# volume-em/empanada-napari

Measured on AMD Instinct MI355X. Metric: EM tiles/sec (1024^2 fp16), higher is better.
Workload: dtype f16

## Files before the change

empanada-napari_amd/csrc/common.h:

```cpp
#pragma once
#include <hip/hip_runtime.h>
#include <stdint.h>
#include <stdio.h>
#include <string>

#include "../../include/empanada_hip.h"

typedef _Float16 half_t;
typedef _Float16 f16x8 __attribute__((ext_vector_type(8)));
typedef _Float16 f16x4 __attribute__((ext_vector_type(4)));
typedef _Float16 f16x2 __attribute__((ext_vector_type(2)));
typedef float f32x4 __attribute__((ext_vector_type(4)));

namespace emp {

void set_error(const char* fmt, ...);

#define EMP_CHECK_HIP(expr)                                                        \
  do {                                                                             \
    hipError_t _e = (expr);                                                        \
    if (_e != hipSuccess) {                                                        \
      emp::set_error("%s:%d: %s -> %s", __FILE__, __LINE__, #expr, hipGetErrorString(_e)); \
      return EMP_ERR_HIP;                                                          \
    }                                                                              \
// ... 22 lines not shown
  const float* bias;
  const float* bias_n;
  const half_t* res;
  half_t* out;
  const half_t* zero;
  int N, H, W, Cin, in_ld;
  int Cout, KH, KW, stride, pad, dil;
  int Ho, Wo, out_ld, res_ld;
  int act;
  int ps_cout;
  int M;
  int mt, nt;
  int mt_per_xcd;
  int kgroup;
  int ngroup;
  const half_t* in2;
  int Cin2, in2_ld, H2, W2, stride2;
  half_t* out2;
  int out2_ld, split;
  half_t* out3;
  int out3_ld, split3;
  const half_t* next_w;
  const float* next_b;
  half_t* next_out;
  int next_cout, next_ld;
};

int launch_conv_igemm(const ConvParams& p, int variant, hipStream_t stream);
int launch_conv_igemm_grouped(const ConvParams& p, int groups, int gs_in, long long gs_w, int gs_out, hipStream_t stream);
bool conv_igemm256_supported(const ConvParams& p);
bool conv_uses_256(const ConvParams& p);
int launch_conv_igemm256(ConvParams p, hipStream_t stream, int kg = 0, int mode = 0, bool wpacked = false);
int conv256_pack_kgroup(int KT, int Cin);
int conv256_pack_weights(const half_t* w, half_t* out, int Cout, int KT, int Cin, int Cin2, hipStream_t stream);
bool conv_b2b_supported(const ConvParams& p);
bool conv_igemm_h256_supported(const ConvParams& p);
int launch_conv_igemm_h256(ConvParams p, hipStream_t stream, int kg = 0);
bool conv_igemm_s64_supported(const ConvParams& p);
int launch_conv_igemm_s64(ConvParams p, hipStream_t stream, int kg = 0);
bool conv3x3_c64_supported(const ConvParams& p);
int launch_conv3x3_c64(const ConvParams& p, hipStream_t stream);

int launch_stem7x7(const void* img, int dtype, float sub, float mul, int N, int H, int W, int vh, int vw,
                   const float* w , const float* b , half_t* out, hipStream_t s);
int launch_maxpool3x3s2(const half_t* in, int N, int H, int W, int C, half_t* out, hipStream_t s);
int launch_stem3x3s2_f16(const void* img, int dtype, float sub, float mul, int N, int H, int W, int vh, int vw,
                         const float* w , const float* b, int C, half_t* out, int out_ld, hipStream_t s);
int launch_gate_mul_f16(const half_t* x, int x_ld, half_t* g , int g_ld, int64_t rows, int C,
                        hipStream_t s);
int launch_stem_pool(const void* img, int dtype, float sub, float mul, int N, int H, int W, int vh, int vw,
                     const float* w, const float* b, half_t* out, hipStream_t s);
int launch_stem_pool_f32(const void* img, int dtype, float sub, float mul, int N, int H, int W, int vh, int vw,
                         const float* w, const float* b, float* out, hipStream_t s);
int launch_dwconv(const half_t* in, int N, int H, int W, int C, int in_ld, const half_t* w, int K,
                  half_t* out, int out_ld, const half_t* zero, hipStream_t s);
int launch_fuse_combine(const half_t* a, const half_t* b, const half_t* c, float ca, float cb, float cc, int mode,
                        int N, int H, int W, int C, half_t* out, hipStream_t s, half_t* out_lo = nullptr, int out_ld = 0);
int launch_bilinear_ac(const half_t* in, int N, int h, int w, int C, int in_ld, half_t* out, int H, int W,
                       int out_ld, hipStream_t s);
int launch_avgpool(const half_t* in, int N, int HW, int C, int in_ld, float* out , float* part,
                   hipStream_t s);
int avgpool_scratch_floats(int N, int C);
int launch_gemv(const float* in, int N, int K, const float* w, const float* b, int Cout, int relu,
                float* out, hipStream_t s);
bool sepconv5_supported(int C, int Cout, int head_c);
int launch_sepconv5_pack_pw(const half_t* w, int pw_ld, int C, int Cout, half_t* packed, hipStream_t s);
// ... 97 lines not shown
```

empanada-napari_amd/csrc/conv_igemm.hip:

```cpp
#include "common.h"

#ifdef EMP_IGEMM_GROUPED
#define EMP_IGEMM_KARGS const ConvParams p_, const int gs_in, const long long gs_w, const int gs_out
#define EMP_IGEMM_KPROLOGUE                                                \
  ConvParams p = p_;                                                       \
  {                                                                        \
    const int g_ = blockIdx.y;                                             \
    p.in += (size_t)g_ * gs_in;                                            \
    p.wgt += (size_t)g_ * (size_t)gs_w;                                    \
    p.out += (size_t)g_ * gs_out;                                          \
    if (p.bias) p.bias += (size_t)g_ * gs_out;                             \
  }
#else
#define EMP_IGEMM_KARGS const ConvParams p
#define EMP_IGEMM_KPROLOGUE
#endif

#include <type_traits>

namespace emp {

namespace {

constexpr int BK = 64;
// ... 387 lines not shown
  ConvParams q = p;
  {
    const int CB = p.Cin / 64, KT = p.KH * p.KW;
    int kg = (KT > 1 && CB > 4 && CB % 4 == 0) ? 4 : CB;
    q.kgroup = kg;
  }
  if (p.Cout <= 64 || cdiv(p.Cout, 64) * 64 <= cdiv(p.Cout, 128) * 128)
    return launch_grouped_tpl<128, 64, 2, 2, true, true, 3>(q, groups, gs_in, gs_w, gs_out, stream);
  return launch_grouped_tpl<128, 128, 2, 2, true, true>(q, groups, gs_in, gs_w, gs_out, stream);
}

#else
template <int BM, int BN, int WPM, int WPN, bool GLDS, bool EPI_LDS, int OCC = 2>
int launch_tpl(ConvParams p, hipStream_t stream) {
  p.mt = cdiv(p.M, BM);
  p.nt = cdiv(p.Cout, BN);
  p.mt_per_xcd = cdiv(p.mt, 8);
  const int grid = 8 * p.mt_per_xcd * p.nt;
  hipLaunchKernelGGL((conv_igemm_kernel<BM, BN, WPM, WPN, GLDS, EPI_LDS, OCC>), dim3(grid), dim3(256), 0, stream, p);
  EMP_LAUNCH_CHECK();
  return EMP_OK;
}

}

bool conv_uses_256(const ConvParams& p) {
  static const bool no256 = [] { const char* e = getenv("EMP_CONV_NO256"); return e && e[0] == '1'; }();
  static const int min_k = [] { const char* e = getenv("EMP_CONV_256_MINK"); return e ? atoi(e) : 512; }();
  const int64_t tiles256 = (int64_t)cdiv(p.M, 256) * (p.Cout / 256);
  const int k256 = p.KH * p.KW * p.Cin + (p.in2 ? p.Cin2 : 0);
  const bool out2_ok = !p.out2 || (!p.out3 && p.split % 256 == 0);
  return !no256 && out2_ok && conv_igemm256_supported(p) && tiles256 >= 192 && k256 >= (p.in2 ? min_k / 4 : min_k);
}
bool conv_uses_h256(const ConvParams& p) {
  static const int h256 = [] { const char* e = getenv("EMP_CONV_H256"); return e ? atoi(e) : 1; }();
  if (!h256 || !conv_igemm_h256_supported(p)) return false;
  const int64_t tiles = (int64_t)cdiv(p.M, 128) * (p.Cout / 128) / 2;
  if (tiles < 1024) return false;
  return h256 == 2 || (p.Cout == 128 && p.KH * p.KW * p.Cin >= 256);
}

int launch_conv_igemm(const ConvParams& p, int variant, hipStream_t stream) {
  EMP_REQUIRE(p.Cin % BK == 0 && p.Cin > 0, "conv: Cin=%d must be a positive multiple of 64", p.Cin);
  EMP_REQUIRE(p.in_ld % 8 == 0 && p.in_ld >= p.Cin, "conv: in_ld=%d must be >= Cin and a multiple of 8", p.in_ld);
  EMP_REQUIRE(p.Cout % 8 == 0 && p.Cout > 0, "conv: Cout=%d must be a positive multiple of 8", p.Cout);
  EMP_REQUIRE(p.out_ld % 8 == 0 && p.out_ld >= (p.ps_cout ? p.ps_cout : (p.out2 ? p.split : p.Cout)), "conv: out_ld=%d invalid", p.out_ld);
  EMP_REQUIRE(p.ps_cout == 0 || (p.ps_cout % 8 == 0 && p.Cout == 4 * p.ps_cout && p.res == nullptr),
              "conv: pixel-shuffle store needs Cout == 4*ps_cout, ps_cout %% 8 == 0, no residual");
  EMP_REQUIRE(p.act >= 0 && p.act <= 2, "conv: act must be 0 (none), 1 (ReLU) or 2 (SiLU)");
  EMP_REQUIRE(p.res == nullptr || p.res_ld % 8 == 0, "conv: res_ld=%d must be a multiple of 8", p.res_ld);
  EMP_REQUIRE(((uintptr_t)p.in % 16) == 0 && ((uintptr_t)p.out % 16) == 0 && ((uintptr_t)p.wgt % 16) == 0 &&
                  ((uintptr_t)p.res % 16) == 0 && ((uintptr_t)p.zero % 256) == 0 && p.zero != nullptr,
              "conv: pointers must be 16-byte aligned (zero page 256)");
  EMP_REQUIRE((int64_t)p.N * p.Ho * p.Wo < (1ll << 31), "conv: too many output pixels");
  if (p.out2) {
    EMP_REQUIRE(p.split > 0 && p.split < p.Cout && p.split % 8 == 0 && p.out2_ld % 8 == 0 &&
                    p.out2_ld >= (p.out3 ? p.split3 : p.Cout) - p.split &&
                    p.out_ld >= p.split && ((uintptr_t)p.out2 % 16) == 0 && p.ps_cout == 0 && p.res == nullptr,
                "conv: second destination: split=%d must be a multiple of 8 inside (0, Cout=%d)", p.split, p.Cout);
  }
  if (p.out3) {
    EMP_REQUIRE(p.out2 != nullptr && p.split3 > p.split && p.split3 < p.Cout && p.split3 % 8 == 0 && p.out3_ld % 8 == 0 &&
                    p.out3_ld >= p.Cout - p.split3 && ((uintptr_t)p.out3 % 16) == 0,
                "conv: third destination: split3=%d must be a multiple of 8 inside (split=%d, Cout=%d)", p.split3, p.split, p.Cout);
  }
  if (p.in2) {
    EMP_REQUIRE(p.KH == 1 && p.KW == 1 && p.stride == 1 && p.pad == 0,
                "conv: a second source needs a 1x1 / stride 1 main convolution");
    EMP_REQUIRE(p.Cin2 > 0 && p.Cin2 % BK == 0 && p.in2_ld % 8 == 0 && p.in2_ld >= p.Cin2 && ((uintptr_t)p.in2 % 16) == 0,
                "conv: second source: Cin2=%d must be a positive multiple of 64, in2_ld=%d >= Cin2", p.Cin2, p.in2_ld);
    EMP_REQUIRE(p.stride2 >= 1 && (p.Ho - 1) * p.stride2 < p.H2 && (p.Wo - 1) * p.stride2 < p.W2,
                "conv: second source %dx%d / stride %d does not cover the %dx%d output", p.H2, p.W2, p.stride2, p.Ho, p.Wo);
  }
  int v = variant & 15, tile = (variant >> 4) & 15, kg = (variant >> 8) & 255, mode256 = (variant >> 16) & 15;
  if ((variant >> 20) & 1) {
    EMP_REQUIRE(!p.next_w && conv_igemm256_supported(p), "conv: packed weights belong to the 256x256 tile");
    return launch_conv_igemm256(p, stream, 0, mode256, true);
  }
  if (p.next_w) {
    EMP_REQUIRE(conv_b2b_supported(p), "conv: a fused next convolution needs the 256x256 tile (Cout == 256, >= 192 tiles)");
    return launch_conv_igemm256(p, stream, kg, mode256);
  }
  EMP_REQUIRE(v <= 3 && tile <= 7, "conv: bad variant %d", variant);
  if (tile == 7) return launch_conv_igemm_s64(p, stream, kg);
  if (tile == 6) return launch_conv3x3_c64(p, stream);
  if (tile == 5) return launch_conv_igemm_h256(p, stream, kg);
  {
    static const bool no_c64 = [] { const char* e = getenv("EMP_CONV_NO_C64"); return e && e[0] == '1'; }();
    if (tile == 0 && !no_c64 && conv3x3_c64_supported(p) && (int64_t)p.N * cdiv(p.H, 8) * cdiv(p.W, 16) >= 1024)
      return launch_conv3x3_c64(p, stream);
  }
  if (tile == 4) {
    return launch_conv_igemm256(p, stream, kg, mode256);
  }
  ConvParams q = p;
  {
    const int CB = p.Cin / 64, KT = p.KH * p.KW;
    static const int env_kg = [] { const char* e = getenv("EMP_CONV_KGROUP"); return e ? atoi(e) : 0; }();
    if (kg == 0) kg = env_kg;
    if (kg == 0) kg = (KT > 1 && CB > 4 && CB % 4 == 0) ? 4 : CB;
    if (kg > CB || CB % kg != 0 || KT == 1) kg = CB;
    q.kgroup = kg;
  }
  if (tile == 0) {
    if (conv_uses_256(p)) return launch_conv_igemm256(p, stream);
    if (conv_uses_h256(p)) return launch_conv_igemm_h256(p, stream);
    tile = (p.Cout <= 64) ? 2 : 1;
    if (p.Cout > 128 && cdiv(p.Cout, 64) * 64 < cdiv(p.Cout, 128) * 128) tile = 2;
    static const int small_below = [] { const char* e = getenv("EMP_CONV_SMALL_TILES_BELOW"); return e ? atoi(e) : 256; }();
// ... 26 lines not shown
```

empanada-napari_amd/csrc/conv_igemm256.hip:

```cpp
#include "common.h"

namespace emp {

namespace {

constexpr int KS = 32;
constexpr int SLOT_BYTES = 512 * 64;
constexpr int W_OFF = 256 * 64;
constexpr int NSLOT = 4;

__device__ __forceinline__ int perm32b(int x) {
  const int t = x >> 4, i = x & 15;
  return ((i >> 2) << 3) + (t << 2) + (i & 3);
}
__device__ __forceinline__ void lds_barrier() {
  asm volatile("s_waitcnt lgkmcnt(0)\n\ts_barrier" ::: "memory");
}

template <int ACT>
__device__ __forceinline__ float act_c(float x) {
  if (ACT == 1) return fmaxf(x, 0.f);
  if (ACT == 2) return x / (1.f + __expf(-x));
  return x;
}
// ... 22 lines not shown
      rv[q][0] = *reinterpret_cast<const f16x8*>(rp);
      rv[q][1] = *reinterpret_cast<const f16x8*>(m < p.M ? rp + 32 : p.zero);
    }
  }
#pragma unroll
  for (int q = 0; q < 8; ++q) {
    const int m = mrow0 + q * 16 + fr;
    if (m >= p.M) continue;
    half_t* orow = (p.out2 && co0 >= p.split) ? p.out2 + (size_t)m * p.out2_ld + (co0 - p.split) + fq * 8
                                              : p.out + (size_t)m * p.out_ld + co0 + fq * 8;
    const float* bn = p.bias_n ? p.bias_n + (size_t)(m / HoWo) * p.Cout + co0 + fq * 8 : nullptr;
#pragma unroll
    for (int P = 0; P < 2; ++P) {
      float v[8];
#pragma unroll
      for (int r = 0; r < 4; ++r) {
        v[r] = acc[2 * P][q][r] + bv[P][r];
        v[4 + r] = acc[2 * P + 1][q][r] + bv[P][4 + r];
      }
      if (bn) {
        const float4 b0 = *reinterpret_cast<const float4*>(bn + P * 32);
        const float4 b1 = *reinterpret_cast<const float4*>(bn + P * 32 + 4);
        v[0] += b0.x; v[1] += b0.y; v[2] += b0.z; v[3] += b0.w;
        v[4] += b1.x; v[5] += b1.y; v[6] += b1.z; v[7] += b1.w;
      }
      if (p.res) {
#pragma unroll
        for (int r = 0; r < 8; ++r) v[r] += (float)rv[q][P][r];
      }
      f16x8 o;
#pragma unroll
      for (int r = 0; r < 8; ++r) o[r] = (half_t)act_c<ACT>(v[r]);
      *reinterpret_cast<f16x8*>(orow + P * 32) = o;
    }
  }
}
template <int ACT>
__device__ __forceinline__ void wave_epilogue_b2b(const ConvParams& p, f32x4 (&acc)[4][8], char* lds, int m0, int grp, int wc,
                                                  int wave, int fr, int fq, int HoWo) {
  const int mrow0 = m0 + grp * 128, co0 = wc * 64;
  float bv[2][8];
#pragma unroll
  for (int P = 0; P < 2; ++P) {
    const int co = co0 + P * 32 + fq * 8;
#pragma unroll
    for (int r = 0; r < 8; ++r) bv[P][r] = 0.f;
    if (p.bias) {
      const float4 b0 = *reinterpret_cast<const float4*>(p.bias + co);
      const float4 b1 = *reinterpret_cast<const float4*>(p.bias + co + 4);
      bv[P][0] = b0.x; bv[P][1] = b0.y; bv[P][2] = b0.z; bv[P][3] = b0.w;
      bv[P][4] = b1.x; bv[P][5] = b1.y; bv[P][6] = b1.z; bv[P][7] = b1.w;
    }
  }
  f16x8 rv[8][2];
  if (p.res) {
#pragma unroll
    for (int q = 0; q < 8; ++q) {
      const int m = mrow0 + q * 16 + fr;
      const half_t* rp = m < p.M ? p.res + (size_t)m * p.res_ld + co0 + fq * 8 : p.zero;
      rv[q][0] = *reinterpret_cast<const f16x8*>(rp);
      rv[q][1] = *reinterpret_cast<const f16x8*>(m < p.M ? rp + 32 : p.zero);
    }
  }
#pragma unroll
  for (int q = 0; q < 8; ++q) {
    const int row = grp * 128 + q * 16 + fr;
// ... 27 lines not shown
#pragma unroll
    for (int tp = 0; tp < 2; ++tp)
#pragma unroll
      for (int t = 0; t < 2; ++t) a2[tp][t] = f32x4{0.f, 0.f, 0.f, 0.f};
    const int r0 = pp * 32 + perm32b(fr), r1 = pp * 32 + perm32b(16 + fr);
#pragma unroll
    for (int ks = 0; ks < 8; ++ks) {
      const f16x8 wa = *reinterpret_cast<const f16x8*>(w2 + r0 * 512 + (((ks * 4 + fq) ^ (r0 & 15)) << 4));
      const f16x8 wb = *reinterpret_cast<const f16x8*>(w2 + r1 * 512 + (((ks * 4 + fq) ^ (r1 & 15)) << 4));
#pragma unroll
      for (int t = 0; t < 2; ++t) {
        const int row = wave * 32 + t * 16 + fr;
        const f16x8 yb = *reinterpret_cast<const f16x8*>(lds + row * 512 + (((ks * 4 + fq) ^ (row & 15)) << 4));
        a2[0][t] = __builtin_amdgcn_mfma_f32_16x16x32_f16(wa, yb, a2[0][t], 0, 0, 0);
        a2[1][t] = __builtin_amdgcn_mfma_f32_16x16x32_f16(wb, yb, a2[1][t], 0, 0, 0);
      }
    }
    const int co2 = pp * 32 + fq * 8;
    const float4 b0 = *reinterpret_cast<const float4*>(p.next_b + co2);
    const float4 b1 = *reinterpret_cast<const float4*>(p.next_b + co2 + 4);
#pragma unroll
    for (int t = 0; t < 2; ++t) {
      const int m = m0 + wave * 32 + t * 16 + fr;
      if (m >= p.M) continue;
      f16x8 o;
      o[0] = (half_t)fmaxf(a2[0][t][0] + b0.x, 0.f); o[1] = (half_t)fmaxf(a2[0][t][1] + b0.y, 0.f);
      o[2] = (half_t)fmaxf(a2[0][t][2] + b0.z, 0.f); o[3] = (half_t)fmaxf(a2[0][t][3] + b0.w, 0.f);
      o[4] = (half_t)fmaxf(a2[1][t][0] + b1.x, 0.f); o[5] = (half_t)fmaxf(a2[1][t][1] + b1.y, 0.f);
      o[6] = (half_t)fmaxf(a2[1][t][2] + b1.z, 0.f); o[7] = (half_t)fmaxf(a2[1][t][3] + b1.w, 0.f);
      *reinterpret_cast<f16x8*>(p.next_out + (size_t)m * p.next_ld + co2) = o;
    }
  }
}
__device__ __forceinline__ void wave_epilogue_any(const ConvParams& p, f32x4 (&acc)[4][8], int mrow0, int co0, int fr,
                                                  int fq, int HoWo) {
  if (p.act == 1) wave_epilogue<1>(p, acc, mrow0, co0, fr, fq, HoWo);
  else if (p.act == 2) wave_epilogue<2>(p, acc, mrow0, co0, fr, fq, HoWo);
  else wave_epilogue<0>(p, acc, mrow0, co0, fr, fq, HoWo);
}

#ifdef EMP_CLOCK_STAMP
__device__ unsigned long long emp_clock_stamp_buf[2 * 8192];
#endif

template <int DMA_EARLY, bool B2B>
__global__ void __launch_bounds__(512, 1) conv_igemm256_kernel(const ConvParams p) {
  extern __shared__ __attribute__((aligned(1024))) char lds[];
#ifdef EMP_CLOCK_STAMP
  const unsigned long long stamp_c0 = __builtin_amdgcn_s_memtime(), stamp_r0 = __builtin_amdgcn_s_memrealtime();
#endif

  const int bid = blockIdx.x;
  const int xcd = bid & 7, j = bid >> 3;
  int mtile = xcd * p.mt_per_xcd + j / p.nt;
  int ntile = j % p.nt;
  if (p.ngroup > 0) {
    const int per = p.mt_per_xcd * p.ngroup, g = j / per, rem = j - g * per;
    mtile = xcd * p.mt_per_xcd + rem / p.ngroup;
    ntile = g * p.ngroup + rem % p.ngroup;
  }
  if (mtile >= p.mt) return;
  const int m0 = mtile * 256, n0 = ntile * 256;

  const int tid = threadIdx.x, l = tid & 63;
  const int wave = __builtin_amdgcn_readfirstlane(tid >> 6);
  const int grp = wave >> 2, wc = wave & 3;
  const int HoWo = p.Ho * p.Wo;
  const int KT = p.KH * p.KW;
// ... 619 lines not shown

  stage();
  if (KTOT > 1) {
    stage();
    asm volatile("s_waitcnt vmcnt(6)" ::: "memory");
  } else {
    asm volatile("s_waitcnt vmcnt(0)" ::: "memory");
  }
  lds_barrier();

  f16x8 pf[8], wf[4];
  for (int t = 0; t < KTOT; ++t) {
    const char* base = lds + (t % 3) * HSLOT;
#pragma unroll
    for (int c = 0; c < 4; ++c) wf[c] = *reinterpret_cast<const f16x8*>(base + w_off + c * 1024);
#pragma unroll
    for (int q = 0; q < 8; ++q) pf[q] = *reinterpret_cast<const f16x8*>(base + p_off + q * 1024);
    if (t + 2 < KTOT) {
      stage();
      asm volatile("s_waitcnt vmcnt(6) lgkmcnt(0)" ::: "memory");
    } else {
      asm volatile("s_waitcnt vmcnt(0) lgkmcnt(0)" ::: "memory");
    }
    __builtin_amdgcn_sched_barrier(0);
    asm volatile("s_barrier" ::: "memory");
    __builtin_amdgcn_s_setprio(1);
#pragma unroll
    for (int q = 0; q < 8; ++q)
#pragma unroll
      for (int c = 0; c < 4; ++c) acc[c][q] = __builtin_amdgcn_mfma_f32_16x16x32_f16(wf[c], pf[q], acc[c][q], 0, 0, 0);
    __builtin_amdgcn_s_setprio(0);
    __builtin_amdgcn_sched_barrier(0);
  }
  wave_epilogue_any(p, acc, m0 + wp * 128, n0 + wc * 64, fr, fq, HoWo);
}

}

bool conv_b2b_supported(const ConvParams& p) {
  return p.next_w != nullptr && p.Cout == 256 && p.next_cout == 64 &&
         p.next_ld % 8 == 0 && p.ps_cout == 0 && p.out2 == nullptr && p.bias_n == nullptr && p.act <= 1 &&
         (int64_t)cdiv(p.M, 256) >= 192 && p.Cin % KS == 0 && (!p.in2 || p.Cin2 % KS == 0);
}

bool conv_igemm256_supported(const ConvParams& p) {
  return p.Cout % 256 == 0 && p.ps_cout == 0 && p.Cin % KS == 0 && p.KH * p.KW * (p.Cin / KS) + (p.in2 ? p.Cin2 / KS : 0) >= 1;
}

__global__ void __launch_bounds__(256) pack256_kernel(const half_t* __restrict__ w, half_t* __restrict__ out, int Cout, int KT,
                                                      int Cin, int Cin2, int KG) {
  const int CB = Cin / KS, KT1 = KT * CB, KTOT = KT1 + Cin2 / KS, Krow = KT * Cin + Cin2;
  const int64_t total = (int64_t)(Cout / 256) * KTOT * 16 * 64;
  for (int64_t i = (int64_t)blockIdx.x * 256 + threadIdx.x; i < total; i += (int64_t)gridDim.x * 256) {
    const int l = (int)(i & 63), pc = (int)((i >> 6) & 15);
    const int64_t tt = i >> 10;
    const int t = (int)(tt % KTOT), ntile = (int)(tt / KTOT);
    const int row = pc * 16 + (l >> 2);
    const int co = ntile * 256 + (row & ~31) + perm32b(row & 31);
    const int chunk = (l & 3) ^ ((-(l >> 4)) & 3);
    int koff;
    if (t < KT1) {
      const int per = KT * KG, g = t / per, idx = t - g * per, tap = idx / KG, cb = idx - tap * KG;
      koff = tap * Cin + (g * KG + cb) * KS;
    } else {
      koff = KT * Cin + (t - KT1) * KS;
    }
    *reinterpret_cast<uint4*>(out + i * 8) = *reinterpret_cast<const uint4*>(w + (size_t)co * Krow + koff + chunk * 8);
  }
}

template <int DMA_EARLY, bool B2B = false>
static int launch256(const ConvParams& p, int grid, hipStream_t stream) {
  constexpr int LDS_BYTES = NSLOT * SLOT_BYTES + (B2B ? 64 * 256 * 2 : 0);
  if (int rc = ensure_dyn_lds(reinterpret_cast<const void*>(&conv_igemm256_kernel<DMA_EARLY, B2B>), LDS_BYTES)) return rc;
  hipLaunchKernelGGL((conv_igemm256_kernel<DMA_EARLY, B2B>), dim3(grid), dim3(512), LDS_BYTES, stream, p);
  EMP_LAUNCH_CHECK();
  return EMP_OK;
}

int launch_conv_igemm256(ConvParams p, hipStream_t stream, int kg, int mode, bool wpacked) {
  EMP_REQUIRE(conv_igemm256_supported(p), "conv256: unsupported shape (Cout=%d)", p.Cout);
  EMP_REQUIRE(p.next_w == nullptr || conv_b2b_supported(p), "conv256: the fused next convolution needs Cout == 256 (got %d)", p.Cout);
  EMP_REQUIRE(p.out2 == nullptr || (p.split % 256 == 0 && p.split > 0 && p.split < p.Cout && p.out3 == nullptr &&
                                    p.next_w == nullptr && p.out2_ld % 8 == 0 && p.out2_ld >= p.Cout - p.split),
              "conv256: a second destination takes whole 256-cout tiles (split=%d)", p.split);
  {
    const int CB = p.Cin / KS, KT = p.KH * p.KW;
    static const int env_kg = [] { const char* e = getenv("EMP_CONV256_KGROUP"); return e ? atoi(e) : 0; }();
    if (kg == 0) kg = env_kg;
    if (kg == 0) kg = 8;
    if (KT == 1 || kg > CB || CB % kg != 0) kg = CB;
    p.kgroup = kg;
  }
  if (wpacked) {
    EMP_REQUIRE(p.next_w == nullptr && p.kgroup == conv256_pack_kgroup(p.KH * p.KW, p.Cin), "conv256: packed weights need the default K walk");
    p.kgroup = -p.kgroup;
  }
  static const int env_mode = [] { const char* e = getenv("EMP_CONV256_MODE"); return e ? atoi(e) : 0; }();
  if (mode == 0) mode = env_mode;
  p.mt = cdiv(p.M, 256);
  p.nt = p.Cout / 256;
  p.mt_per_xcd = cdiv(p.mt, 8);
  {
    static const int env_ng = [] { const char* e = getenv("EMP_CONV256_NGROUP"); return e ? atoi(e) : 0; }();
    p.ngroup = (env_ng > 0 && p.KH * p.KW == 1 && p.nt >= 2 * env_ng && p.nt % env_ng == 0 && !p.next_w) ? env_ng : 0;
  }
  const int grid = 8 * p.mt_per_xcd * p.nt;
  if (p.next_w) return launch256<0, true>(p, grid, stream);
  {
    static const bool wide_on = [] { const char* e = getenv("EMP_CONV256_WIDE"); return !(e && e[0] == '0'); }();
    const int kga = p.kgroup < 0 ? -p.kgroup : p.kgroup;
    const int ktot = p.KH * p.KW * (p.Cin / KS) + (p.in2 ? p.Cin2 / KS : 0);
    if (wide_on && mode == 0 && p.Cin % (2 * KS) == 0 && (!p.in2 || p.Cin2 % (2 * KS) == 0) && kga % 2 == 0 && ktot >= 8 &&
        (int64_t)p.N * p.H * p.W < (1ll << 31)) {
      if (int rc = ensure_dyn_lds(reinterpret_cast<const void*>(&conv_igemm256w_kernel), WIDE_LDS_BYTES)) return rc;
      hipLaunchKernelGGL(conv_igemm256w_kernel, dim3(grid), dim3(512), WIDE_LDS_BYTES, stream, p);
      EMP_LAUNCH_CHECK();
      return EMP_OK;
    }
  }
  if (mode == 1) return launch256<2>(p, grid, stream);
  if (mode == 2) return launch256<4>(p, grid, stream);
  return launch256<0>(p, grid, stream);
}

int conv256_pack_kgroup(int KT, int Cin) {
  const int CB = Cin / KS;
  static const int env_kg = [] { const char* e = getenv("EMP_CONV256_KGROUP"); return e ? atoi(e) : 0; }();
  int kg = env_kg ? env_kg : 8;
  if (KT == 1 || kg > CB || CB % kg != 0) kg = CB;
  return kg;
}
int conv256_pack_weights(const half_t* w, half_t* out, int Cout, int KT, int Cin, int Cin2, hipStream_t stream) {
  EMP_REQUIRE(w && out && Cout > 0 && Cout % 256 == 0 && Cin > 0 && Cin % KS == 0 && Cin2 >= 0 && Cin2 % KS == 0 && KT >= 1,
              "conv256_pack_weights: bad shape (Cout=%d Cin=%d Cin2=%d)", Cout, Cin, Cin2);
  const int64_t chunks = (int64_t)Cout * (KT * Cin + Cin2) / 8;
  hipLaunchKernelGGL(pack256_kernel, dim3((unsigned)std::min<int64_t>((chunks + 255) / 256, 4096)), dim3(256), 0, stream, w, out, Cout,
                     KT, Cin, Cin2, conv256_pack_kgroup(KT, Cin));
  EMP_LAUNCH_CHECK();
  return EMP_OK;
}

bool conv_igemm_h256_supported(const ConvParams& p) {
  return p.Cout % 128 == 0 && p.ps_cout == 0 && p.out2 == nullptr && p.Cin % KS == 0 && (!p.in2 || p.Cin2 % KS == 0);
}

template <int PXR, int COR>
static int launch_h256(ConvParams p, hipStream_t stream) {
  constexpr int LDS_BYTES = 3 * (PXR + COR) * 64;
  if (int rc = ensure_dyn_lds(reinterpret_cast<const void*>(&conv_igemm_h256_kernel<PXR, COR>), LDS_BYTES)) return rc;
  p.mt = cdiv(p.M, PXR);
  p.nt = p.Cout / COR;
  p.mt_per_xcd = cdiv(p.mt, 8);
  const int grid = 8 * p.mt_per_xcd * p.nt;
  hipLaunchKernelGGL((conv_igemm_h256_kernel<PXR, COR>), dim3(grid), dim3(256), LDS_BYTES, stream, p);
  EMP_LAUNCH_CHECK();
  return EMP_OK;
}

int launch_conv_igemm_h256(ConvParams p, hipStream_t stream, int kg) {
  EMP_REQUIRE(conv_igemm_h256_supported(p), "conv h256: unsupported shape (Cout=%d)", p.Cout);
  const int CB = p.Cin / KS, KT = p.KH * p.KW;
  if (kg == 0) kg = 8;
  if (KT == 1 || kg > CB || CB % kg != 0) kg = CB;
  p.kgroup = kg;
  if (p.Cout % 256 == 0) return launch_h256<128, 256>(p, stream);
  return launch_h256<256, 128>(p, stream);
}

// ... 9 lines not shown
```

empanada-napari_amd/csrc/pdl_net.hip:

```cpp
#include <string.h>

#include <array>
#include <map>
#include <memory>
#include <string>
#include <vector>

#include "common.h"

namespace emp {

namespace {

struct HostParam {
  std::vector<int64_t> shape;
  std::vector<float> w, b;
  bool set = false;
};

struct Act {
  half_t* p = nullptr;
  int N = 0, H = 0, W = 0, C = 0, ld = 0;
  size_t off = 0;
};

struct DevConv {
  half_t* w = nullptr;
  half_t* w256 = nullptr;
  float* b = nullptr;
  int cout = 0, cin = 0, cin_pad = 0, kh = 1, kw = 1;
  int cin2 = 0, cin2_pad = 0;
  bool wsplit = false;
};

inline int round_up(int a, int b) { return (a + b - 1) / b * b; }

}
}

using namespace emp;

struct emp_pdl {
  emp_pdl_config cfg;
  int aspp_ch = 256, dec_ch = 256, ncls = 1;
  std::vector<std::string> param_names;
  std::map<std::string, HostParam> params;
  bool finalized = false;
  FILE* layer_log = [] { const char* e = getenv("EMP_LAYER_LOG"); return e ? fopen(e, "w") : (FILE*)nullptr; }();
  bool fuse_stem = [] { const char* e = getenv("EMP_FUSE_STEM"); return !(e && e[0] == '0'); }();
  bool fuse_ds = [] { const char* e = getenv("EMP_FUSE_DS"); return !(e && e[0] == '0'); }();
  bool fuse_b2b = [] { const char* e = getenv("EMP_FUSE_B2B"); return !(e && e[0] == '0'); }();
  bool pack256 = [] { const char* e = getenv("EMP_CONV256_PACK"); return !(e && e[0] == '0'); }();
  bool fuse_proj = [] { const char* e = getenv("EMP_FUSE_PROJ"); return !(e && e[0] == '0'); }();
  bool fuse_aspp = [] { const char* e = getenv("EMP_FUSE_ASPP"); return !(e && e[0] == '0'); }();
  bool fuse_sepconv = [] { const char* e = getenv("EMP_FUSE_SEPCONV"); return !(e && e[0] == '0'); }();
  bool fuse_pr = [] { const char* e = getenv("EMP_FUSE_PR"); return !(e && e[0] == '0'); }();
  int precise_sepconv = [] { const char* e = getenv("EMP_PRECISE_SEPCONV"); return e ? atoi(e) : 1; }();
  bool precise_wsplit = [] { const char* e = getenv("EMP_PRECISE_WSPLIT"); return !(e && e[0] == '0'); }();
  bool precise_fsplit = [] { const char* e = getenv("EMP_PRECISE_FSPLIT"); return !(e && e[0] == '0'); }();
  int sepconv_min_tiles = [] { const char* e = getenv("EMP_SEPCONV_MIN_TILES"); return e ? atoi(e) : 256; }();

  int precision = [] {
    const char* e = getenv("EMP_PRECISION");
    if (e && (!strcmp(e, "fp16") || !strcmp(e, "16"))) return 0;
    if (e && (!strcmp(e, "fp32") || !strcmp(e, "32"))) return 1;
    return 2;
  }();
  bool fp32_graph() const { return precision != 0; }
  bool x3_fuse_ds = [] { const char* e = getenv("EMP_X3_FUSE_DS"); return !(e && e[0] == '0'); }();
  bool x3_fuse_head = [] { const char* e = getenv("EMP_X3_FUSE_HEAD"); return !(e && e[0] == '0'); }();
  bool x3_planes = [] { const char* e = getenv("EMP_X3_PLANES"); return !(e && e[0] == '0'); }();
  int x3_planes_min_tiles = [] { const char* e = getenv("EMP_X3_PLANES_MIN_TILES"); return e ? atoi(e) : 128; }();
  bool x3_planes_ready = false;
  bool x3_ksplit = [] { const char* e = getenv("EMP_X3_KSPLIT"); return !(e && e[0] == '0'); }();
  float* x3_kpart = nullptr;
  bool x3_small_aspp = [] { const char* e = getenv("EMP_X3_SMALL_ASPP"); return !(e && e[0] == '0'); }();
  bool x3_fuse_stem = [] { const char* e = getenv("EMP_X3_FUSE_STEM"); return !(e && e[0] == '0'); }();
  bool x3_merge_proj = [] { const char* e = getenv("EMP_X3_MERGE_PROJ"); return !(e && e[0] == '0'); }();
  bool x3_merge_aspp = [] { const char* e = getenv("EMP_X3_MERGE_ASPP"); return !(e && e[0] == '0'); }();
  bool x3_fuse_sep = [] { const char* e = getenv("EMP_X3_FUSE_SEP"); return !(e && e[0] == '0'); }();
  int x3_sep_min_tiles = [] { const char* e = getenv("EMP_X3_SEP_MIN_TILES"); return e ? atoi(e) : 1; }();
  struct SepX3 { float* dw = nullptr; half_t* pw = nullptr; int C = 0, Cout = 0, ks = 0; };
  std::map<std::string, SepX3> sepx3;
  bool regnet_grouped = [] { const char* e = getenv("EMP_REGNET_GROUPED"); return !(e && e[0] == '0'); }();
  int64_t regnet_group_tiles = [] { const char* e = getenv("EMP_REGNET_GROUP_TILES"); return e ? atoll(e) : 2048ll; }();
// ... 593 lines not shown
  p.N = in.N; p.H = in.H; p.W = in.W; p.Cin = dc.cin_pad; p.in_ld = in.ld;
  p.Cout = dc.cout; p.KH = dc.kh; p.KW = dc.kw; p.stride = stride; p.pad = pad; p.dil = dil;
  p.Ho = (in.H + 2 * pad - dil * (dc.kh - 1) - 1) / stride + 1;
  p.Wo = (in.W + 2 * pad - dil * (dc.kw - 1) - 1) / stride + 1;
  const int up = ps_cout ? 2 : 1;
  EMP_REQUIRE(p.Ho * up == out.H && p.Wo * up == out.W && in.N == out.N, "%s: output shape mismatch (%dx%d vs %dx%d)",
              wname.c_str(), p.Ho * up, p.Wo * up, out.H, out.W);
  EMP_REQUIRE(in_coff + dc.cin_pad <= in.ld && out_coff + (ps_cout ? ps_cout : (out2 ? split : dc.cout)) <= out.ld,
              "%s: channel slice out of range", wname.c_str());
  p.out_ld = out.ld;
  p.act = act;
  p.ps_cout = ps_cout;
  p.M = p.N * p.Ho * p.Wo;
  double next_flops = 0.0;
  if (fused_next) *fused_next = false;
  if (next_name && n->fuse_b2b) {
    const DevConv& nd = n->convs.at(*next_name);
    p.next_w = nd.w; p.next_b = nd.b; p.next_out = next_out->p; p.next_cout = nd.cout; p.next_ld = next_out->ld;
    if (nd.kh == 1 && nd.kw == 1 && nd.cin_pad == dc.cout && nd.cin2_pad == 0 && next_out->N == out.N && next_out->H == out.H &&
        next_out->W == out.W && nd.cout <= next_out->ld && out_coff == 0 && conv_b2b_supported(p)) {
      *fused_next = true;
      next_flops = 2.0 * (double)p.M * nd.cout * (double)nd.cin;
      n->flops += next_flops;
    } else {
      p.next_w = nullptr; p.next_b = nullptr; p.next_out = nullptr; p.next_cout = 0; p.next_ld = 0;
    }
  }
  const double kflop = (double)(dc.cin * dc.kh * dc.kw + (dc.wsplit ? 0 : dc.cin2));
  n->flops += 2.0 * (double)p.M * dc.cout * kflop;
  if (n->layer_log)
    fprintf(n->layer_log, "conv,%s,%d,%d,%d,%d,%d,%d,%d,%d\n", wname.c_str(), p.M, dc.cin_pad + dc.cin2_pad, dc.cout, dc.kh,
            stride, dil, res ? 1 : 0, in.N * in.H * in.W);
  int variant = 0;
  if (n->pack256 && !p.next_w && conv_uses_256(p)) {
    if (dc.w256) {
      p.wgt = dc.w256;
      variant = 1 << 20;
    }
  }
  if (n->profile && !p.next_w && conv_uses_256(p)) {
    if (n->prof_used == n->prof_events.size()) {
      hipEvent_t a, b;
      EMP_CHECK_HIP(hipEventCreate(&a));
      EMP_CHECK_HIP(hipEventCreate(&b));
      n->prof_events.emplace_back(a, b);
    }
    auto& ev = n->prof_events[n->prof_used++];
    EMP_CHECK_HIP(hipEventRecord(ev.first, s));
    const int rc = launch_conv_igemm(p, variant, s);
    EMP_CHECK_HIP(hipEventRecord(ev.second, s));
    n->prof_flops += 2.0 * (double)p.M * dc.cout * kflop;
    return rc;
  }
  return launch_conv_igemm(p, variant, s);
}

#define RC(x)            \
  do {                   \
    int _rc = (x);       \
    if (_rc) return _rc; \
  } while (0)

int run(emp_pdl* n, const void* img, int dtype, float sub, float mul, int N, int H, int W, int vh, int vw, int RS,
        int interp, float* o_sem, float* o_ctr, float* o_off, hipStream_t s) {
  const emp_pdl_config& c = n->cfg;
  n->flops = 0.0;
  auto A = [&](const std::string& k) -> Act& { return n->acts.at(k); };
// ... 1594 lines not shown
          rc = pack_conv(n, tm);
          n->params.erase(tm);
          if (rc) return rc;
        }
      }
    }
  }
  const char* heads[3] = {"semantic_head", "ins_center", "ins_xy"};
  for (int k = 0; k < 3; ++k) {
    std::string p = heads[k];
    RC(pack_dw(n, p + ".head.0.0.sepconv.0", n->dec_ch));
    RC(pack_conv(n, p + ".head.0.0.sepconv.1"));
    RC(pack_sepconv_pw(n, p + ".head.0.0.sepconv.1"));
    if (precise_layer(n, p + ".head.0.0")) RC(pack_sepconvp_pw(n, p + ".head.0.0.sepconv.1"));
    RC(upload_f32(n, p + ".head.1.w", n->params[p + ".head.1"].w));
    RC(upload_f32(n, p + ".head.1.b", n->params[p + ".head.1"].b));
  }
  const int ldp = round_up(n->dec_ch + n->ncls, 64);
  for (int k = 0; k < c.num_fc; ++k) RC(pack_conv(n, "semantic_pr.point_head.fc_layers." + std::to_string(k) + ".0", ldp));
  {
    const HostParam& hp = n->params["semantic_pr.point_head.predictor"];
    const int K = (int)hp.shape[1];
    std::vector<float> w((size_t)n->ncls * ldp, 0.f);
    for (int o = 0; o < n->ncls; ++o)
      for (int i = 0; i < K; ++i) w[(size_t)o * ldp + i] = hp.w[(size_t)o * K + i];
    RC(upload_f32(n, "pr.predictor.w", w));
    RC(upload_f32(n, "pr.predictor.b", hp.b));
  }
  if (n->fp32_graph()) RC(finalize32(n));
  if (n->pack256 && !n->fp32_graph()) {
    for (auto& kv : n->convs) {
      DevConv& dc = kv.second;
      const int K = dc.kh * dc.kw * dc.cin_pad + dc.cin2_pad;
      if (dc.w256 || !dc.w || dc.cout % 256 != 0 || dc.cin_pad % 64 != 0 || dc.cin2_pad % 64 != 0 || K < (dc.cin2_pad ? 128 : 512)) continue;
      const size_t halfs = (size_t)dc.cout * K;
      EMP_CHECK_HIP(hipMalloc((void**)&dc.w256, halfs * sizeof(half_t)));
      n->owned.push_back(dc.w256);
      n->image_bytes += halfs * sizeof(half_t);
      const int prc = conv256_pack_weights(dc.w, dc.w256, dc.cout, dc.kh * dc.kw, dc.cin_pad, dc.cin2_pad, nullptr);
      if (prc) return prc;
    }
    EMP_CHECK_HIP(hipStreamSynchronize(nullptr));
  }
  n->finalized = true;
  return EMP_OK;
}

int emp_pdl_set_precision(emp_pdl_t* net, int precision) {
  EMP_REQUIRE(net, "set_precision: null network");
  EMP_REQUIRE(precision >= 0 && precision <= 2, "set_precision: 0 = fp16 engine, 1 = fp32 reference mode, 2 = fp16x3 mode (got %d)", precision);
  EMP_REQUIRE(!net->finalized, "set_precision: call before emp_pdl_finalize");
  net->precision = precision;
  return EMP_OK;
}
int emp_pdl_precision(const emp_pdl_t* net) { return net ? net->precision : -1; }

int emp_pdl_reserve(emp_pdl_t* net, int N, int H, int W) {
  EMP_REQUIRE(net, "reserve: null network");
  if (net->fp32_graph()) return EMP_OK;
  return plan(net, N, H, W, net->pRS > 2 ? net->pRS : 2, nullptr);
}
size_t emp_pdl_arena_bytes(const emp_pdl_t* net) { return net ? net->arena_used : 0; }

int emp_pdl_forward_padded(emp_pdl_t* net, const void* d_image, int image_dtype, float sub, float mul, int N, int vh, int vw,
                           int H, int W, int render_steps, int interpolate_ins, float* d_sem_logits, float* d_ctr_hmp,
                           float* d_offsets, void* stream) {
  EMP_REQUIRE(net && d_image && d_sem_logits && d_ctr_hmp && d_offsets, "forward: null argument");
  EMP_REQUIRE(vh > 0 && vw > 0 && vh <= H && vw <= W, "forward: valid size %dx%d must fit the padded size %dx%d", vh, vw, H, W);
// ... 85 lines not shown
```

Before: 1332.

## Route three-destination 1x1 convs with partial-256 Cout through packed 256x256 kernel

Extends the 256x256 implicit-GEMM conv path to 1x1 convolutions whose Cout is between 129 and 256 and not a multiple of 256, and which write to up to three output buffers. Weights are packed zero-padded to a full 256-column tile, and a new per-column epilogue picks the destination buffer and skips out-of-range channels. The intent is to run fused multi-head 1x1 convs on the faster large-tile kernel instead of the generic igemm. The cost is wasted MMA work on the zero-padded columns and a more branchy epilogue.

```diff
diff --git a/empanada-napari_amd/csrc/common.h b/empanada-napari_amd/csrc/common.h
--- a/empanada-napari_amd/csrc/common.h
+++ b/empanada-napari_amd/csrc/common.h
@@ -78,6 +78,10 @@
 bool conv_uses_256(const ConvParams& p);
 int launch_conv_igemm256(ConvParams p, hipStream_t stream, int kg = 0, int mode = 0, bool wpacked = false);
 int conv256_pack_kgroup(int KT, int Cin);
+int64_t conv256_image_halfs(int Cout, int K);
+bool conv256_multi_shape(int Cout, int KT, int Cin, int Cin2);
+bool conv_igemm256_multi_supported(const ConvParams& p);
+bool conv_uses_256_multi(const ConvParams& p);
 int conv256_pack_weights(const half_t* w, half_t* out, int Cout, int KT, int Cin, int Cin2, hipStream_t stream);
 bool conv_b2b_supported(const ConvParams& p);
 bool conv_igemm_h256_supported(const ConvParams& p);
diff --git a/empanada-napari_amd/csrc/conv_igemm.hip b/empanada-napari_amd/csrc/conv_igemm.hip
--- a/empanada-napari_amd/csrc/conv_igemm.hip
+++ b/empanada-napari_amd/csrc/conv_igemm.hip
@@ -443,6 +443,9 @@
   const bool out2_ok = !p.out2 || (!p.out3 && p.split % 256 == 0);
   return !no256 && out2_ok && conv_igemm256_supported(p) && tiles256 >= 192 && k256 >= (p.in2 ? min_k / 4 : min_k);
 }
+bool conv_uses_256_multi(const ConvParams& p) {
+  return p.out2 && p.out3 && conv_igemm256_multi_supported(p) && (int64_t)cdiv(p.M, 256) >= 192;
+}
 bool conv_uses_h256(const ConvParams& p) {
   static const int h256 = [] { const char* e = getenv("EMP_CONV_H256"); return e ? atoi(e) : 1; }();
   if (!h256 || !conv_igemm_h256_supported(p)) return false;
@@ -485,7 +488,8 @@
   }
   int v = variant & 15, tile = (variant >> 4) & 15, kg = (variant >> 8) & 255, mode256 = (variant >> 16) & 15;
   if ((variant >> 20) & 1) {
-    EMP_REQUIRE(!p.next_w && conv_igemm256_supported(p), "conv: packed weights belong to the 256x256 tile");
+    EMP_REQUIRE(!p.next_w && (conv_igemm256_supported(p) || conv_igemm256_multi_supported(p)),
+                "conv: packed weights belong to the 256x256 tile");
     return launch_conv_igemm256(p, stream, 0, mode256, true);
   }
   if (p.next_w) {
diff --git a/empanada-napari_amd/csrc/conv_igemm256.hip b/empanada-napari_amd/csrc/conv_igemm256.hip
--- a/empanada-napari_amd/csrc/conv_igemm256.hip
+++ b/empanada-napari_amd/csrc/conv_igemm256.hip
@@ -78,6 +78,45 @@
 #pragma unroll
       for (int r = 0; r < 8; ++r) o[r] = (half_t)act_c<ACT>(v[r]);
       *reinterpret_cast<f16x8*>(orow + P * 32) = o;
+    }
+  }
+}
+template <int ACT>
+__device__ __forceinline__ void wave_epilogue_multi(const ConvParams& p, f32x4 (&acc)[4][8], int mrow0, int co0, int fr, int fq) {
+#pragma unroll
+  for (int P = 0; P < 2; ++P) {
+    const int co = co0 + P * 32 + fq * 8;
+    if (co >= p.Cout) continue;
+    float bv[8];
+#pragma unroll
+    for (int r = 0; r < 8; ++r) bv[r] = 0.f;
+    if (p.bias) {
+      const float4 b0 = *reinterpret_cast<const float4*>(p.bias + co);
+      const float4 b1 = *reinterpret_cast<const float4*>(p.bias + co + 4);
+      bv[0] = b0.x; bv[1] = b0.y; bv[2] = b0.z; bv[3] = b0.w;
+      bv[4] = b1.x; bv[5] = b1.y; bv[6] = b1.z; bv[7] = b1.w;
+    }
+    half_t* dst = p.out + co;
+    int dld = p.out_ld;
+    if (p.out2 && co >= p.split) {
+      dst = p.out2 + (co - p.split);
+      dld = p.out2_ld;
+      if (p.out3 && co >= p.split3) {
+        dst = p.out3 + (co - p.split3);
+        dld = p.out3_ld;
+      }
+    }
+#pragma unroll
+    for (int q = 0; q < 8; ++q) {
+      const int m = mrow0 + q * 16 + fr;
+      if (m >= p.M) continue;
+      f16x8 o;
+#pragma unroll
+      for (int r = 0; r < 4; ++r) {
+        o[r] = (half_t)act_c<ACT>(acc[2 * P][q][r] + bv[r]);
+        o[4 + r] = (half_t)act_c<ACT>(acc[2 * P + 1][q][r] + bv[4 + r]);
+      }
+      *reinterpret_cast<f16x8*>(dst + (size_t)m * dld) = o;
     }
   }
 }
@@ -171,8 +210,15 @@
     }
   }
 }
+template <bool MULTI = true>
 __device__ __forceinline__ void wave_epilogue_any(const ConvParams& p, f32x4 (&acc)[4][8], int mrow0, int co0, int fr,
                                                   int fq, int HoWo) {
+  if (MULTI && (p.out3 || (p.Cout & 255) || (p.out2 && (p.split & 255)))) {
+    if (p.act == 1) wave_epilogue_multi<1>(p, acc, mrow0, co0, fr, fq);
+    else if (p.act == 2) wave_epilogue_multi<2>(p, acc, mrow0, co0, fr, fq);
+    else wave_epilogue_multi<0>(p, acc, mrow0, co0, fr, fq);
+    return;
+  }
   if (p.act == 1) wave_epilogue<1>(p, acc, mrow0, co0, fr, fq, HoWo);
   else if (p.act == 2) wave_epilogue<2>(p, acc, mrow0, co0, fr, fq, HoWo);
   else wave_epilogue<0>(p, acc, mrow0, co0, fr, fq, HoWo);
@@ -858,7 +904,7 @@
     __builtin_amdgcn_s_setprio(0);
     __builtin_amdgcn_sched_barrier(0);
   }
-  wave_epilogue_any(p, acc, m0 + wp * 128, n0 + wc * 64, fr, fq, HoWo);
+  wave_epilogue_any<false>(p, acc, m0 + wp * 128, n0 + wc * 64, fr, fq, HoWo);
 }
 
 }
@@ -872,11 +918,18 @@
 bool conv_igemm256_supported(const ConvParams& p) {
   return p.Cout % 256 == 0 && p.ps_cout == 0 && p.Cin % KS == 0 && p.KH * p.KW * (p.Cin / KS) + (p.in2 ? p.Cin2 / KS : 0) >= 1;
 }
+bool conv256_multi_shape(int Cout, int KT, int Cin, int Cin2) {
+  return KT == 1 && Cin2 == 0 && Cout > 128 && Cout <= 256 && Cout % 8 == 0 && Cin % 64 == 0 && Cin >= 256;
+}
+bool conv_igemm256_multi_supported(const ConvParams& p) {
+  return conv256_multi_shape(p.Cout, p.KH * p.KW, p.Cin, p.in2 ? p.Cin2 : 0) && p.stride == 1 && p.pad == 0 && p.ps_cout == 0 &&
+         p.res == nullptr && p.bias_n == nullptr && p.next_w == nullptr;
+}
 
 __global__ void __launch_bounds__(256) pack256_kernel(const half_t* __restrict__ w, half_t* __restrict__ out, int Cout, int KT,
                                                       int Cin, int Cin2, int KG) {
   const int CB = Cin / KS, KT1 = KT * CB, KTOT = KT1 + Cin2 / KS, Krow = KT * Cin + Cin2;
-  const int64_t total = (int64_t)(Cout / 256) * KTOT * 16 * 64;
+  const int64_t total = (int64_t)((Cout + 255) / 256) * KTOT * 16 * 64;
   for (int64_t i = (int64_t)blockIdx.x * 256 + threadIdx.x; i < total; i += (int64_t)gridDim.x * 256) {
     const int l = (int)(i & 63), pc = (int)((i >> 6) & 15);
     const int64_t tt = i >> 10;
@@ -891,7 +944,8 @@
     } else {
       koff = KT * Cin + (t - KT1) * KS;
     }
-    *reinterpret_cast<uint4*>(out + i * 8) = *reinterpret_cast<const uint4*>(w + (size_t)co * Krow + koff + chunk * 8);
+    *reinterpret_cast<uint4*>(out + i * 8) =
+        co < Cout ? *reinterpret_cast<const uint4*>(w + (size_t)co * Krow + koff + chunk * 8) : uint4{0u, 0u, 0u, 0u};
   }
 }
 
@@ -905,11 +959,24 @@
 }
 
 int launch_conv_igemm256(ConvParams p, hipStream_t stream, int kg, int mode, bool wpacked) {
-  EMP_REQUIRE(conv_igemm256_supported(p), "conv256: unsupported shape (Cout=%d)", p.Cout);
-  EMP_REQUIRE(p.next_w == nullptr || conv_b2b_supported(p), "conv256: the fused next convolution needs Cout == 256 (got %d)", p.Cout);
-  EMP_REQUIRE(p.out2 == nullptr || (p.split % 256 == 0 && p.split > 0 && p.split < p.Cout && p.out3 == nullptr &&
-                                    p.next_w == nullptr && p.out2_ld % 8 == 0 && p.out2_ld >= p.Cout - p.split),
-              "conv256: a second destination takes whole 256-cout tiles (split=%d)", p.split);
+  const bool multi = p.Cout % 256 != 0 || p.out3 != nullptr || (p.out2 != nullptr && p.split % 256 != 0);
+  if (multi) {
+    EMP_REQUIRE(wpacked && conv_igemm256_multi_supported(p),
+                "conv256: Cout=%d / %d destinations need the packed weight image and a plain epilogue (no residual, no per-image bias)",
+                p.Cout, 1 + (p.out2 != nullptr) + (p.out3 != nullptr));
+    EMP_REQUIRE(p.out2 == nullptr || (p.split % 8 == 0 && p.split > 0 && p.split < p.Cout && p.out2_ld % 8 == 0 &&
+                                      p.out2_ld >= (p.out3 ? p.split3 : p.Cout) - p.split),
+                "conv256: second destination: split=%d must be a multiple of 8 inside (0, Cout=%d)", p.split, p.Cout);
+    EMP_REQUIRE(p.out3 == nullptr || (p.out2 != nullptr && p.split3 % 8 == 0 && p.split3 > p.split && p.split3 < p.Cout &&
+                                      p.out3_ld % 8 == 0 && p.out3_ld >= p.Cout - p.split3),
+                "conv256: third destination: split3=%d must be a multiple of 8 inside (split=%d, Cout=%d)", p.split3, p.split, p.Cout);
+  } else {
+    EMP_REQUIRE(conv_igemm256_supported(p), "conv256: unsupported shape (Cout=%d)", p.Cout);
+    EMP_REQUIRE(p.next_w == nullptr || conv_b2b_supported(p), "conv256: the fused next convolution needs Cout == 256 (got %d)", p.Cout);
+    EMP_REQUIRE(p.out2 == nullptr || (p.split > 0 && p.split < p.Cout && p.next_w == nullptr && p.out2_ld % 8 == 0 &&
+                                      p.out2_ld >= p.Cout - p.split),
+                "conv256: a second destination takes whole 256-cout tiles (split=%d)", p.split);
+  }
   {
     const int CB = p.Cin / KS, KT = p.KH * p.KW;
     static const int env_kg = [] { const char* e = getenv("EMP_CONV256_KGROUP"); return e ? atoi(e) : 0; }();
@@ -925,7 +992,7 @@
   static const int env_mode = [] { const char* e = getenv("EMP_CONV256_MODE"); return e ? atoi(e) : 0; }();
   if (mode == 0) mode = env_mode;
   p.mt = cdiv(p.M, 256);
-  p.nt = p.Cout / 256;
+  p.nt = cdiv(p.Cout, 256);
   p.mt_per_xcd = cdiv(p.mt, 8);
   {
     static const int env_ng = [] { const char* e = getenv("EMP_CONV256_NGROUP"); return e ? atoi(e) : 0; }();
@@ -957,10 +1024,12 @@
   if (KT == 1 || kg > CB || CB % kg != 0) kg = CB;
   return kg;
 }
+int64_t conv256_image_halfs(int Cout, int K) { return (int64_t)cdiv(Cout, 256) * 256 * K; }
 int conv256_pack_weights(const half_t* w, half_t* out, int Cout, int KT, int Cin, int Cin2, hipStream_t stream) {
-  EMP_REQUIRE(w && out && Cout > 0 && Cout % 256 == 0 && Cin > 0 && Cin % KS == 0 && Cin2 >= 0 && Cin2 % KS == 0 && KT >= 1,
+  EMP_REQUIRE(w && out && Cout > 0 && (Cout % 256 == 0 || conv256_multi_shape(Cout, KT, Cin, Cin2)) && Cin > 0 && Cin % KS == 0 &&
+                  Cin2 >= 0 && Cin2 % KS == 0 && KT >= 1,
               "conv256_pack_weights: bad shape (Cout=%d Cin=%d Cin2=%d)", Cout, Cin, Cin2);
-  const int64_t chunks = (int64_t)Cout * (KT * Cin + Cin2) / 8;
+  const int64_t chunks = conv256_image_halfs(Cout, KT * Cin + Cin2) / 8;
   hipLaunchKernelGGL(pack256_kernel, dim3((unsigned)std::min<int64_t>((chunks + 255) / 256, 4096)), dim3(256), 0, stream, w, out, Cout,
                      KT, Cin, Cin2, conv256_pack_kgroup(KT, Cin));
   EMP_LAUNCH_CHECK();
diff --git a/empanada-napari_amd/csrc/pdl_net.hip b/empanada-napari_amd/csrc/pdl_net.hip
--- a/empanada-napari_amd/csrc/pdl_net.hip
+++ b/empanada-napari_amd/csrc/pdl_net.hip
@@ -51,6 +51,7 @@
   bool fuse_ds = [] { const char* e = getenv("EMP_FUSE_DS"); return !(e && e[0] == '0'); }();
   bool fuse_b2b = [] { const char* e = getenv("EMP_FUSE_B2B"); return !(e && e[0] == '0'); }();
   bool pack256 = [] { const char* e = getenv("EMP_CONV256_PACK"); return !(e && e[0] == '0'); }();
+  bool multi256 = [] { const char* e = getenv("EMP_CONV_MULTI256"); return !(e && e[0] == '0'); }();
   bool fuse_proj = [] { const char* e = getenv("EMP_FUSE_PROJ"); return !(e && e[0] == '0'); }();
   bool fuse_aspp = [] { const char* e = getenv("EMP_FUSE_ASPP"); return !(e && e[0] == '0'); }();
   bool fuse_sepconv = [] { const char* e = getenv("EMP_FUSE_SEPCONV"); return !(e && e[0] == '0'); }();
@@ -710,7 +711,7 @@
     fprintf(n->layer_log, "conv,%s,%d,%d,%d,%d,%d,%d,%d,%d\n", wname.c_str(), p.M, dc.cin_pad + dc.cin2_pad, dc.cout, dc.kh,
             stride, dil, res ? 1 : 0, in.N * in.H * in.W);
   int variant = 0;
-  if (n->pack256 && !p.next_w && conv_uses_256(p)) {
+  if (n->pack256 && !p.next_w && (conv_uses_256(p) || (n->multi256 && conv_uses_256_multi(p)))) {
     if (dc.w256) {
       p.wgt = dc.w256;
       variant = 1 << 20;
@@ -2371,8 +2372,9 @@
     for (auto& kv : n->convs) {
       DevConv& dc = kv.second;
       const int K = dc.kh * dc.kw * dc.cin_pad + dc.cin2_pad;
-      if (dc.w256 || !dc.w || dc.cout % 256 != 0 || dc.cin_pad % 64 != 0 || dc.cin2_pad % 64 != 0 || K < (dc.cin2_pad ? 128 : 512)) continue;
-      const size_t halfs = (size_t)dc.cout * K;
+      const bool whole = dc.cout % 256 == 0 && dc.cin_pad % 64 == 0 && dc.cin2_pad % 64 == 0 && K >= (dc.cin2_pad ? 128 : 512);
+      if (dc.w256 || !dc.w || !(whole || conv256_multi_shape(dc.cout, dc.kh * dc.kw, dc.cin_pad, dc.cin2_pad))) continue;
+      const size_t halfs = (size_t)conv256_image_halfs(dc.cout, K);
       EMP_CHECK_HIP(hipMalloc((void**)&dc.w256, halfs * sizeof(half_t)));
       n->owned.push_back(dc.w256);
       n->image_bytes += halfs * sizeof(half_t);
```

Result: no change. 1336, median of 6 (+0.3%).
